# tyfeld/MMaDA-Parallel

Hardware: NVIDIA H100
Metric: denoised_tokens_per_sec (higher is better)
Workload: dtype bf16; 1 GPU; MMaDA-Parallel-A 8B, 1 prompt per GPU, 512x512 (1024 VQ tokens) + 256 text tokens, timesteps=64, text_steps=128, cfg_img=4.0, cfg_scale=0, temperature=1.0, text_temperature=0 (BASELINE configs[1]); seq_len=2414, parallelism=replicas x1 (independent prompts, no collective), weights=synthetic normal(0, 0.02) bf16, seeded, l2=16.2 GB of weights streamed per forward >> 50 MB L2 (no flush needed)

## Files before the change

mmada_parallel_b200/csrc/attention.cu:

```cuda
#include "mmdp_internal.h"
#include "ptx.cuh"

#include <stdlib.h>

#include <map>
#include <mutex>
#include <utility>

namespace mmdp {

static constexpr int kAttnThreads = 384;
static constexpr int kQBytes = 128 * 128 * 2;
template <int BKV> struct AttnCfg {
    static constexpr int kKBytes = BKV * 128 * 2;
    static constexpr int kVBytes = 128 * BKV * 2;
    static constexpr int kSmem = kQBytes + 2 * (kKBytes + kVBytes) + 1024  + 256 ;
};

__device__ __forceinline__ float ex2_approx(float x) {
    float y;
    asm("ex2.approx.ftz.f32 %0, %1;" : "=f"(y) : "f"(x));
    return y;
}

struct AttnSegs {
    int n;
    int start[kMaxSegs + 1];
    int tile0[kMaxSegs + 1];
};

struct AttnWin {
    AttnSegs segs;
    int q0[kMaxSegs], nq[kMaxSegs], out0[kMaxSegs];
};

template <int kBKV, bool kPacked, bool kGqa = false, bool kWin = false>
__device__ __forceinline__ void attention_body(const CUtensorMap& tmQ, const CUtensorMap& tmK, const CUtensorMap& tmVt,
                                               __nv_bfloat16* __restrict__ out, int H, int L, int d_model, float scale_log2,
                                               int n_full, int splits, float* __restrict__ part_ws, int Lq, const AttnSegs* segs,
                                               int kv_group = 1, const AttnWin* win = nullptr) {
    constexpr int kKBytes = AttnCfg<kBKV>::kKBytes, kVBytes = AttnCfg<kBKV>::kVBytes;
    extern __shared__ uint8_t smem_raw[];
    uint8_t* smem = reinterpret_cast<uint8_t*>((reinterpret_cast<uintptr_t>(smem_raw) + 1023) & ~uintptr_t(1023));
    uint8_t* sQ = smem;
    uint8_t* sK = sQ + kQBytes;
    uint8_t* sV = sK + 2 * kKBytes;
    uint64_t* bars = reinterpret_cast<uint64_t*>(sV + 2 * kVBytes);
    uint64_t* q_full = bars + 0;
    uint64_t* k_full = bars + 1;
    uint64_t* k_empty = bars + 3;
    uint64_t* v_full = bars + 5;
    uint64_t* v_empty = bars + 7;

    const int warp = threadIdx.x >> 5, lane = threadIdx.x & 31, wg = warp >> 2;
    int n_qt = (Lq + 127) / 128;
    int n_kv_all = (L + kBKV - 1) / kBKV;
    int tile = blockIdx.x, piece = -1;
    if ((int)blockIdx.x >= n_full) {
        const int t = (int)blockIdx.x - n_full;
        tile = n_full + t / splits;
        piece = t - (t / splits) * splits;
    }
    int seg = 0, seg0 = 0, tl = tile, q0 = 0, o0 = 0;
    if constexpr (kPacked) {
        for (int i = 1; i < segs->n; ++i)
            if (tile >= segs->tile0[i]) seg = i;
        seg0 = segs->start[seg];
        L = Lq = segs->start[seg + 1] - seg0;
        o0 = seg0;
        if constexpr (kWin) {
            q0 = win->q0[seg];
            Lq = win->nq[seg];
            o0 = win->out0[seg];
        }
        n_qt = (Lq + 127) / 128;
        n_kv_all = (L + kBKV - 1) / kBKV;
        tl = tile - segs->tile0[seg];
    }
    const int qt = tl % n_qt, h = (tl / n_qt) % H, b = kPacked ? seg : tile / (n_qt * H);
    const int hk = kGqa ? h / kv_group : h, Hk = kGqa ? H / kv_group : H;
    int jb = 0, je = n_kv_all;
    if (piece >= 0) {
        const int per = (n_kv_all + splits - 1) / splits;
        jb = piece * per;
        je = (jb + per < n_kv_all) ? jb + per : n_kv_all;
    }
    const int n_kv = je - jb;

    if (warp == 0 && lane == 0) {
        tma_prefetch_desc(&tmQ);
        tma_prefetch_desc(&tmK);
        tma_prefetch_desc(&tmVt);
        mbar_init(q_full, 1);
        for (int s = 0; s < 2; ++s) {
            mbar_init(&k_full[s], 1);
            mbar_init(&k_empty[s], 8);
            mbar_init(&v_full[s], 1);
            mbar_init(&v_empty[s], 8);
        }
        fence_barrier_init();
    }
    __syncthreads();
    pdl_launch_dependents();
    pdl_wait();

    if (wg == 0) {
        setmaxnreg_dec<40>();
        if (warp == 0 && elect_one_sync()) {
            const int qrow0 = (kPacked ? seg0 + q0 : b * Lq) + qt * 128;
            mbar_expect_tx(q_full, kQBytes);
            tma_load_2d(sQ, &tmQ, q_full, h * 128, qrow0);
            tma_load_2d(sQ + kQBytes / 2, &tmQ, q_full, h * 128 + 64, qrow0);
            for (int j = 0; j < n_kv; ++j) {
                const int st = j & 1;
                const uint32_t ph = (j >> 1) & 1;
                const int kv0 = (jb + j) * kBKV;
                mbar_wait(&k_empty[st], ph ^ 1);
                mbar_expect_tx(&k_full[st], kKBytes);
                tma_load_2d(sK + st * kKBytes, &tmK, &k_full[st], hk * 128, (kPacked ? seg0 : b * L) + kv0);
                tma_load_2d(sK + st * kKBytes + kKBytes / 2, &tmK, &k_full[st], hk * 128 + 64, (kPacked ? seg0 : b * L) + kv0);
                mbar_wait(&v_empty[st], ph ^ 1);
                mbar_expect_tx(&v_full[st], kVBytes);
                tma_load_2d(sV + st * kVBytes, &tmVt, &v_full[st], kv0, (b * Hk + hk) * 128);
                if (kBKV == 128) tma_load_2d(sV + st * kVBytes + kVBytes / 2, &tmVt, &v_full[st], kv0 + 64, (b * Hk + hk) * 128);
            }
        }
        __syncwarp();
        return;
    }

    setmaxnreg_inc<232>();
    const int half = wg - 1;
    const int r0 = half * 64 + (warp & 3) * 16 + (lane >> 2), c0 = 2 * (lane & 3);
    const uint32_t aQ = smem_u32(sQ) + half * (64 * 128);
    float o[64];
#pragma unroll
    for (int i = 0; i < 64; ++i) o[i] = 0.f;
    float m_run[2] = {-INFINITY, -INFINITY}, l_run[2] = {0.f, 0.f};
    mbar_wait(q_full, 0);
    for (int j = 0; j < n_kv; ++j) {
        const int st = j & 1;
        const uint32_t ph = (j >> 1) & 1;
        const int nvalid = L - (jb + j) * kBKV;
        float sacc[kBKV / 2];
        const uint32_t aK = smem_u32(sK + st * kKBytes);
        mbar_wait(&k_full[st], ph);
        wgmma_fence();
#pragma unroll
        for (int kk = 0; kk < 8; ++kk)
        {
            const uint64_t qd = smem_desc_kmajor_sw128(aQ + (kk >> 2) * (kQBytes / 2)) + (kk & 3) * 2;
            const uint64_t kd = smem_desc_kmajor_sw128(aK + (kk >> 2) * (kKBytes / 2)) + (kk & 3) * 2;
            if constexpr (kBKV == 128) wgmma_bf16_ss_n128(sacc, qd, kd, kk != 0);
            else wgmma_bf16_ss_n64(sacc, qd, kd, kk != 0);
        }
        wgmma_commit();
        wgmma_wait<0>();
        reg_fence(sacc);
        __syncwarp();
        if (lane == 0) mbar_arrive(&k_empty[st]);
        if (nvalid < kBKV) {
#pragma unroll
            for (int jj = 0; jj < kBKV / 8; ++jj)
#pragma unroll
                for (int e = 0; e < 2; ++e)
                    if (8 * jj + c0 + e >= nvalid) { sacc[4 * jj + e] = -INFINITY; sacc[4 * jj + 2 + e] = -INFINITY; }
        }
        float alpha[2], mneg[2];
#pragma unroll
        for (int hh = 0; hh < 2; ++hh) {
            float mx = sacc[2 * hh];
#pragma unroll
            for (int jj = 0; jj < kBKV / 8; ++jj) mx = fmaxf(mx, fmaxf(sacc[4 * jj + 2 * hh], sacc[4 * jj + 2 * hh + 1]));
            mx = fmaxf(mx, __shfl_xor_sync(0xffffffffu, mx, 1));
            mx = fmaxf(mx, __shfl_xor_sync(0xffffffffu, mx, 2));
            const float m_new = fmaxf(m_run[hh], mx);
            alpha[hh] = ex2_approx((m_run[hh] - m_new) * scale_log2);
            m_run[hh] = m_new;
            mneg[hh] = -m_new * scale_log2;
        }
        uint32_t pa[kBKV / 4];
        float rsum[2] = {0.f, 0.f};
#pragma unroll
        for (int jj = 0; jj < kBKV / 8; ++jj)
#pragma unroll
            for (int hh = 0; hh < 2; ++hh) {
                const float p0 = ex2_approx(fmaf(sacc[4 * jj + 2 * hh], scale_log2, mneg[hh]));
                const float p1 = ex2_approx(fmaf(sacc[4 * jj + 2 * hh + 1], scale_log2, mneg[hh]));
                rsum[hh] += p0 + p1;
                pa[2 * jj + hh] = pack_bf16x2(p0, p1);
            }
#pragma unroll
        for (int hh = 0; hh < 2; ++hh) l_run[hh] = fmaf(l_run[hh], alpha[hh], rsum[hh]);
#pragma unroll
        for (int jj = 0; jj < 16; ++jj) {
            o[4 * jj] *= alpha[0]; o[4 * jj + 1] *= alpha[0];
            o[4 * jj + 2] *= alpha[1]; o[4 * jj + 3] *= alpha[1];
        }
        const uint32_t aV = smem_u32(sV + st * kVBytes);
        mbar_wait(&v_full[st], ph);
        wgmma_fence();
#pragma unroll
        for (int kk = 0; kk < kBKV / 16; ++kk) {
            const uint32_t a[4] = {pa[4 * kk], pa[4 * kk + 1], pa[4 * kk + 2], pa[4 * kk + 3]};
            wgmma_bf16_rs_n128(o, a, smem_desc_kmajor_sw128(aV + (kk >> 2) * (kVBytes / 2)) + (kk & 3) * 2, 1);
        }
        wgmma_commit();
        wgmma_wait<0>();
        reg_fence(o);
        __syncwarp();
        if (lane == 0) mbar_arrive(&v_empty[st]);
    }
#pragma unroll
    for (int hh = 0; hh < 2; ++hh) {
        l_run[hh] += __shfl_xor_sync(0xffffffffu, l_run[hh], 1);
        l_run[hh] += __shfl_xor_sync(0xffffffffu, l_run[hh], 2);
    }
#pragma unroll
    for (int hh = 0; hh < 2; ++hh) {
        const int r = r0 + 8 * hh, qrow = qt * 128 + r;
        if (qrow >= Lq) continue;
        if (piece >= 0) {
            float* slot = part_ws + (size_t)((tile - n_full) * splits + piece) * (128 * 128 + 256);
            if ((lane & 3) == 0) {
                slot[128 * 128 + r] = m_run[hh];
                slot[128 * 128 + 128 + r] = l_run[hh];
            }
#pragma unroll
            for (int jj = 0; jj < 16; ++jj)
                *reinterpret_cast<float2*>(slot + (size_t)r * 128 + 8 * jj + c0) = make_float2(o[4 * jj + 2 * hh], o[4 * jj + 2 * hh + 1]);
        } else {
            const float inv_l = 1.0f / l_run[hh];
            __nv_bfloat16* orow = out + (size_t)((kPacked ? o0 : b * Lq) + qrow) * d_model + h * 128;
#pragma unroll
            for (int jj = 0; jj < 16; ++jj)
                *reinterpret_cast<uint32_t*>(orow + 8 * jj + c0) = pack_bf16x2(o[4 * jj + 2 * hh] * inv_l, o[4 * jj + 2 * hh + 1] * inv_l);
        }
    }
}

template <int kBKV>
__global__ void __launch_bounds__(kAttnThreads, 1)
attention_kernel(const __grid_constant__ CUtensorMap tmQ, const __grid_constant__ CUtensorMap tmK,
                 const __grid_constant__ CUtensorMap tmVt, __nv_bfloat16* __restrict__ out, int H, int L, int d_model,
                 float scale_log2, int n_full, int splits, float* __restrict__ part_ws, int Lq) {
    attention_body<kBKV, false>(tmQ, tmK, tmVt, out, H, L, d_model, scale_log2, n_full, splits, part_ws, Lq, nullptr);
}

template <int kBKV>
__global__ void __launch_bounds__(kAttnThreads, 1)
attention_packed_kernel(const __grid_constant__ CUtensorMap tmQ, const __grid_constant__ CUtensorMap tmK,
                        const __grid_constant__ CUtensorMap tmVt, __nv_bfloat16* __restrict__ out, int H, int d_model,
                        float scale_log2, int n_full, int splits, float* __restrict__ part_ws, const __grid_constant__ AttnSegs segs) {
    attention_body<kBKV, true>(tmQ, tmK, tmVt, out, H, 0, d_model, scale_log2, n_full, splits, part_ws, 0, &segs);
}

template <int kBKV>
__global__ void __launch_bounds__(kAttnThreads, 1)
attention_gqa_kernel(const __grid_constant__ CUtensorMap tmQ, const __grid_constant__ CUtensorMap tmK,
                     const __grid_constant__ CUtensorMap tmVt, __nv_bfloat16* __restrict__ out, int H, int L, int d_model,
                     float scale_log2, int n_full, int splits, float* __restrict__ part_ws, int Lq, int kv_group) {
    attention_body<kBKV, false, true>(tmQ, tmK, tmVt, out, H, L, d_model, scale_log2, n_full, splits, part_ws, Lq, nullptr, kv_group);
}

template <int kBKV>
__global__ void __launch_bounds__(kAttnThreads, 1)
attention_packed_gqa_kernel(const __grid_constant__ CUtensorMap tmQ, const __grid_constant__ CUtensorMap tmK,
                            const __grid_constant__ CUtensorMap tmVt, __nv_bfloat16* __restrict__ out, int H, int d_model,
                            float scale_log2, int n_full, int splits, float* __restrict__ part_ws, const __grid_constant__ AttnSegs segs,
                            int kv_group) {
    attention_body<kBKV, true, true>(tmQ, tmK, tmVt, out, H, 0, d_model, scale_log2, n_full, splits, part_ws, 0, &segs, kv_group);
}

template <int kBKV, bool kGqa>
__global__ void __launch_bounds__(kAttnThreads, 1)
attention_packed_window_kernel(const __grid_constant__ CUtensorMap tmQ, const __grid_constant__ CUtensorMap tmK,
                               const __grid_constant__ CUtensorMap tmVt, __nv_bfloat16* __restrict__ out, int H, int d_model,
                               float scale_log2, int n_full, int splits, float* __restrict__ part_ws, const __grid_constant__ AttnWin win,
                               int kv_group) {
    attention_body<kBKV, true, kGqa, true>(tmQ, tmK, tmVt, out, H, 0, d_model, scale_log2, n_full, splits, part_ws, 0, &win.segs,
                                           kv_group, &win);
}

template <bool kPacked, bool kWin = false>
__device__ __forceinline__ void attention_combine_body(const float* __restrict__ part_ws, __nv_bfloat16* __restrict__ out, int H,
                                                       int Lq, int d_model, float scale_log2, int n_full, int splits,
                                                       const AttnSegs* segs, const AttnWin* win = nullptr) {
    int n_qt = (Lq + 127) / 128;
    const int st = blockIdx.x, r = blockIdx.y, c = threadIdx.x;
    pdl_launch_dependents();
    pdl_wait();
    const int tile = n_full + st;
    int seg = 0, seg0 = 0, tl = tile;
    if constexpr (kPacked) {
        for (int i = 1; i < segs->n; ++i)
            if (tile >= segs->tile0[i]) seg = i;
        seg0 = segs->start[seg];
        Lq = segs->start[seg + 1] - seg0;
        if constexpr (kWin) {
            seg0 = win->out0[seg];
            Lq = win->nq[seg];
        }
        n_qt = (Lq + 127) / 128;
        tl = tile - segs->tile0[seg];
    }
    const int qt = tl % n_qt, h = (tl / n_qt) % H, b = kPacked ? seg : tile / (n_qt * H);
    const int qrow = qt * 128 + r;
    if (qrow >= Lq) return;
    const float* base = part_ws + (size_t)st * splits * (128 * 128 + 256);
    float m = -INFINITY;
    for (int i = 0; i < splits; ++i) m = fmaxf(m, base[(size_t)i * (128 * 128 + 256) + 128 * 128 + r]);
    float o = 0.f, l = 0.f;
    for (int i = 0; i < splits; ++i) {
        const float* slot = base + (size_t)i * (128 * 128 + 256);
        const float w = exp2f((slot[128 * 128 + r] - m) * scale_log2);
        o = fmaf(w, slot[(size_t)r * 128 + c], o);
        l = fmaf(w, slot[128 * 128 + 128 + r], l);
    }
    out[(size_t)((kPacked ? seg0 : b * Lq) + qrow) * d_model + h * 128 + c] = __float2bfloat16_rn(o / l);
}

__global__ void __launch_bounds__(128)
attention_combine_kernel(const float* __restrict__ part_ws, __nv_bfloat16* __restrict__ out, int H, int Lq, int d_model,
                         float scale_log2, int n_full, int splits) {
    attention_combine_body<false>(part_ws, out, H, Lq, d_model, scale_log2, n_full, splits, nullptr);
}

__global__ void __launch_bounds__(128)
attention_packed_combine_kernel(const float* __restrict__ part_ws, __nv_bfloat16* __restrict__ out, int H, int d_model,
                                float scale_log2, int n_full, int splits, const __grid_constant__ AttnSegs segs) {
    attention_combine_body<true>(part_ws, out, H, 0, d_model, scale_log2, n_full, splits, &segs);
}

__global__ void __launch_bounds__(128)
attention_packed_window_combine_kernel(const float* __restrict__ part_ws, __nv_bfloat16* __restrict__ out, int H, int d_model,
                                       float scale_log2, int n_full, int splits, const __grid_constant__ AttnWin win) {
    attention_combine_body<true, true>(part_ws, out, H, 0, d_model, scale_log2, n_full, splits, &win.segs, &win);
}

static std::map<std::pair<int, cudaStream_t>, std::pair<float*, size_t>> g_attn_ws;
static std::mutex g_attn_ws_mu;
static int attn_part_workspace(cudaStream_t stream, size_t need, float** out) {
    int dev = 0;
    MMDP_CUDA(cudaGetDevice(&dev));
    std::lock_guard<std::mutex> lk(g_attn_ws_mu);
    auto& e = g_attn_ws[std::make_pair(dev, stream)];
    if (need > e.second) {
        if (e.first) MMDP_CUDA(cudaFree(e.first));
        e.first = nullptr; e.second = 0;
        MMDP_CUDA(cudaMalloc(&e.first, need));
        e.second = need;
    }
    *out = e.first;
    return 0;
}

template <class KvbOf>
static void plan_split_tail(int tiles, KvbOf kvb_of, int& n_full, int& n_split, int& splits) {
    const int split_tail = opt(OPT_ATTN_SPLIT_TAIL), slots = num_sms();
    n_full = tiles; n_split = 0; splits = 1;
    auto fit_splits = [&](int want, int first) {
        int sp = want > 8 ? 8 : want;
        for (int t = first; t < tiles; ++t)
            if (sp > kvb_of(t) / 2) sp = kvb_of(t) / 2;
        auto empty_piece = [&](int s) {
            for (int t = first; t < tiles; ++t) {
                const int n_kvb = kvb_of(t);
                if ((s - 1) * ((n_kvb + s - 1) / s) >= n_kvb) return true;
            }
            return false;
        };
        while (sp >= 2 && empty_piece(sp)) --sp;
        return sp;
    };
    if (split_tail && tiles > slots && (tiles % slots) > 0 && (tiles % slots) * 4 <= slots) {
        n_split = tiles % slots;
        splits = fit_splits(slots / n_split, tiles - n_split);
        if (splits >= 2) n_full = tiles - n_split; else { n_split = 0; splits = 1; }
    } else if (split_tail && tiles * 2 <= slots) {
        splits = fit_splits(slots / tiles, 0);
        if (splits >= 2) { n_split = tiles; n_full = 0; } else splits = 1;
    }
}

template <class Kernel>
static int attn_smem_attr(Kernel kernel, int smem, unsigned long long& attr_set) {
    int dev = 0;
    MMDP_CUDA(cudaGetDevice(&dev));
    if (!(attr_set >> (dev & 63) & 1ull)) {
        MMDP_CUDA(cudaFuncSetAttribute(kernel, cudaFuncAttributeMaxDynamicSharedMemorySize, smem));
        attr_set |= 1ull << (dev & 63);
    }
    return 0;
}

template <int kBKV>
static int attention_launch(const __nv_bfloat16* q, const __nv_bfloat16* k, const __nv_bfloat16* vt, __nv_bfloat16* out, int B, int H,
                            int L, int Lpad, float scale, cudaStream_t stream, int Lq, int Hkv) {
    constexpr int kAttnSmem = AttnCfg<kBKV>::kSmem;
    if (B <= 0 || H <= 0 || L <= 0) return set_error("attention: empty problem");
    if (Lq <= 0) Lq = L;
    if (Hkv <= 0) Hkv = H;
    if (Hkv > H || H % Hkv) return set_error("attention: n_kv_heads=%d must divide n_heads=%d", Hkv, H);
    if (Lpad < L || (Lpad % 8)) return set_error("attention: Lpad must be >= L and a multiple of 8");
    const int d_model = H * 128, d_kv = Hkv * 128;
    CUtensorMap tmQ, tmK, tmVt;
    if (make_tmap_2d_bf16(&tmQ, q, (uint64_t)B * Lq, (uint64_t)d_model, (uint64_t)d_model, 128, 64)) return -1;
    if (make_tmap_2d_bf16(&tmK, k, (uint64_t)B * L, (uint64_t)d_kv, (uint64_t)d_kv, kBKV, 64)) return -1;
    if (make_tmap_2d_bf16(&tmVt, vt, (uint64_t)B * Hkv * 128, (uint64_t)Lpad, (uint64_t)Lpad, 128, 64)) return -1;
    const int n_qt = (Lq + 127) / 128, n_kvb = (L + kBKV - 1) / kBKV;
    const int tiles = n_qt * H * B;
    int n_full, n_split, splits;
    plan_split_tail(tiles, [&](int) { return n_kvb; }, n_full, n_split, splits);
    float* part_ws = nullptr;
    if (n_split > 0 && attn_part_workspace(stream, (size_t)n_split * splits * (128 * 128 + 256) * sizeof(float), &part_ws)) return -1;
    const int grid = n_full + n_split * splits;
    const float scale_log2 = scale * 1.4426950408889634f;
    const bool pdl = pdl_mode() != 0;
    LaunchScope ls(LK_ATTN, 4.0 * B * H * (double)Lq * L * 128, stream);
    if (Hkv != H) {
        static unsigned long long attr_set_gqa = 0;
        if (attn_smem_attr(attention_gqa_kernel<kBKV>, kAttnSmem, attr_set_gqa)) return -1;
        MMDP_CUDA(launch_ex(attention_gqa_kernel<kBKV>, dim3(grid), dim3(kAttnThreads), kAttnSmem, stream, pdl, false, tmQ, tmK, tmVt, out,
                            H, L, d_model, scale_log2, n_full, splits, part_ws, Lq, H / Hkv));
    } else {
        static unsigned long long attr_set = 0;
        if (attn_smem_attr(attention_kernel<kBKV>, kAttnSmem, attr_set)) return -1;
        MMDP_CUDA(launch_ex(attention_kernel<kBKV>, dim3(grid), dim3(kAttnThreads), kAttnSmem, stream, pdl, false, tmQ, tmK, tmVt, out, H, L,
                            d_model, scale_log2, n_full, splits, part_ws, Lq));
    }
    if (n_split > 0)
        MMDP_CUDA(launch_ex(attention_combine_kernel, dim3(n_split, 128), dim3(128), 0, stream, pdl, false, (const float*)part_ws, out, H, Lq,
                            d_model, scale_log2, n_full, splits));
    return 0;
}

template <int kBKV>
static int attention_packed_launch(const __nv_bfloat16* q, const __nv_bfloat16* k, const __nv_bfloat16* vt, __nv_bfloat16* out,
                                   const SegTable& segs, int H, int Lpad, float scale, cudaStream_t stream, int Hkv,
                                   const int* win_lo, const int* win_hi) {
    constexpr int kAttnSmem = AttnCfg<kBKV>::kSmem;
    if (segs.n <= 0 || segs.n > kMaxSegs || H <= 0) return set_error("attention_packed: %d sequences (1 to %d)", segs.n, kMaxSegs);
    if (Hkv <= 0) Hkv = H;
    if (Hkv > H || H % Hkv) return set_error("attention_packed: n_kv_heads=%d must divide n_heads=%d", Hkv, H);
    if (Lpad % 8) return set_error("attention_packed: Lpad must be a multiple of 8");
    if (!win_lo != !win_hi) return set_error("attention_packed: give both window bounds or neither");
    const bool windowed = win_lo != nullptr;
    AttnWin aw{};
    AttnSegs& as = aw.segs;
    as.n = segs.n;
    double work = 0;
    int Mq = 0;
    for (int s = 0; s <= segs.n; ++s) {
        as.start[s] = segs.start[s];
        if (s == segs.n) break;
        const int len = segs.start[s + 1] - segs.start[s];
        if (len <= 0 || len > Lpad) return set_error("attention_packed: sequence %d has length %d (Lpad %d)", s, len, Lpad);
        const int lo = windowed ? win_lo[s] : 0, hi = windowed ? win_hi[s] : len;
        if (lo < 0 || lo >= hi || hi > len)
            return set_error("attention_packed: sequence %d of length %d has the row window [%d, %d)", s, len, lo, hi);
        aw.q0[s] = lo;
        aw.nq[s] = hi - lo;
        aw.out0[s] = Mq;
        Mq += hi - lo;
        as.tile0[s + 1] = as.tile0[s] + (hi - lo + 127) / 128 * H;
        work += 4.0 * H * (double)(hi - lo) * len * 128;
    }
    const int M = segs.start[segs.n], tiles = as.tile0[segs.n], d_model = H * 128, d_kv = Hkv * 128;
    CUtensorMap tmQ, tmK, tmVt;
    if (make_tmap_2d_bf16(&tmQ, q, (uint64_t)M, (uint64_t)d_model, (uint64_t)d_model, 128, 64)) return -1;
    if (make_tmap_2d_bf16(&tmK, k, (uint64_t)M, (uint64_t)d_kv, (uint64_t)d_kv, kBKV, 64)) return -1;
    if (make_tmap_2d_bf16(&tmVt, vt, (uint64_t)segs.n * Hkv * 128, (uint64_t)Lpad, (uint64_t)Lpad, 128, 64)) return -1;
    auto kvb_of = [&](int t) {
        int s = 0;
        while (s + 1 < segs.n && t >= as.tile0[s + 1]) ++s;
        return (segs.start[s + 1] - segs.start[s] + kBKV - 1) / kBKV;
    };
    int n_full, n_split, splits;
    plan_split_tail(tiles, kvb_of, n_full, n_split, splits);
    float* part_ws = nullptr;
    if (n_split > 0 && attn_part_workspace(stream, (size_t)n_split * splits * (128 * 128 + 256) * sizeof(float), &part_ws)) return -1;
    const int grid = n_full + n_split * splits;
    const float scale_log2 = scale * 1.4426950408889634f;
    const bool pdl = pdl_mode() != 0;
    LaunchScope ls(LK_ATTN, work, stream);
    if (windowed) {
        auto kernel = Hkv != H ? attention_packed_window_kernel<kBKV, true> : attention_packed_window_kernel<kBKV, false>;
        static unsigned long long attr_set_win[2] = {0, 0};
        if (attn_smem_attr(kernel, kAttnSmem, attr_set_win[Hkv != H])) return -1;
        MMDP_CUDA(launch_ex(kernel, dim3(grid), dim3(kAttnThreads), kAttnSmem, stream, pdl, false, tmQ, tmK, tmVt, out, H, d_model,
                            scale_log2, n_full, splits, part_ws, aw, H / Hkv));
        if (n_split > 0)
            MMDP_CUDA(launch_ex(attention_packed_window_combine_kernel, dim3(n_split, 128), dim3(128), 0, stream, pdl, false,
                                (const float*)part_ws, out, H, d_model, scale_log2, n_full, splits, aw));
        return 0;
    }
    if (Hkv != H) {
        static unsigned long long attr_set_gqa = 0;
        if (attn_smem_attr(attention_packed_gqa_kernel<kBKV>, kAttnSmem, attr_set_gqa)) return -1;
        MMDP_CUDA(launch_ex(attention_packed_gqa_kernel<kBKV>, dim3(grid), dim3(kAttnThreads), kAttnSmem, stream, pdl, false, tmQ, tmK, tmVt,
                            out, H, d_model, scale_log2, n_full, splits, part_ws, as, H / Hkv));
    } else {
        static unsigned long long attr_set = 0;
        if (attn_smem_attr(attention_packed_kernel<kBKV>, kAttnSmem, attr_set)) return -1;
        MMDP_CUDA(launch_ex(attention_packed_kernel<kBKV>, dim3(grid), dim3(kAttnThreads), kAttnSmem, stream, pdl, false, tmQ, tmK, tmVt, out,
                            H, d_model, scale_log2, n_full, splits, part_ws, as));
    }
    if (n_split > 0)
        MMDP_CUDA(launch_ex(attention_packed_combine_kernel, dim3(n_split, 128), dim3(128), 0, stream, pdl, false, (const float*)part_ws,
                            out, H, d_model, scale_log2, n_full, splits, as));
    return 0;
}

int attention_fwd(const __nv_bfloat16* q, const __nv_bfloat16* k, const __nv_bfloat16* vt, __nv_bfloat16* out, int B, int H, int L,
                  int Lpad, float scale, cudaStream_t stream, int Lq, int Hkv) {
    const int version = opt(OPT_ATTN_VERSION);
    if (version == 7) return attention_launch<64>(q, k, vt, out, B, H, L, Lpad, scale, stream, Lq, Hkv);
    if (version != 6) return set_error("attention: unknown kernel generation %d (6 or 7)", version);
    return attention_launch<128>(q, k, vt, out, B, H, L, Lpad, scale, stream, Lq, Hkv);
}

int attention_packed_fwd(const __nv_bfloat16* q, const __nv_bfloat16* k, const __nv_bfloat16* vt, __nv_bfloat16* out,
                         const SegTable& segs, int H, int Lpad, float scale, cudaStream_t stream, int Hkv, const int* win_lo,
                         const int* win_hi) {
    const int version = opt(OPT_ATTN_VERSION);
    if (version == 7) return attention_packed_launch<64>(q, k, vt, out, segs, H, Lpad, scale, stream, Hkv, win_lo, win_hi);
    if (version != 6) return set_error("attention: unknown kernel generation %d (6 or 7)", version);
    return attention_packed_launch<128>(q, k, vt, out, segs, H, Lpad, scale, stream, Hkv, win_lo, win_hi);
}

}
```

mmada_parallel_b200/csrc/mmdp_internal.h:

```cpp
#pragma once
#include <cuda.h>
#include <cuda_bf16.h>
#include <cuda_runtime.h>
#include <stdint.h>
#include <stdio.h>

namespace mmdp {

enum Epilogue { EPI_PLAIN = 0, EPI_RESID = 1, EPI_QKVROPE = 2, EPI_SWIGLU = 3, EPI_F32 = 4, EPI_QKVROPE_PACKED = 5,
                EPI_QKVGQA = 6, EPI_QKVGQA_PACKED = 7 };
constexpr bool epi_is_gqa(int epi) { return epi == EPI_QKVGQA || epi == EPI_QKVGQA_PACKED; }
constexpr bool epi_is_qkv(int epi) { return epi == EPI_QKVROPE || epi == EPI_QKVROPE_PACKED || epi_is_gqa(epi); }
constexpr bool epi_is_packed(int epi) { return epi == EPI_QKVROPE_PACKED || epi == EPI_QKVGQA_PACKED; }

static constexpr int kMaxSegs = 64;
struct SegTable {
    int n;
    int start[kMaxSegs + 1];
};

int set_error(const char* fmt, ...);
const char* last_error();
int num_sms();

enum LaunchKind { LK_GEMM = 0, LK_ATTN = 1, LK_ROW = 2, LK_SAMPLE = 3, LK_COUNT = 4 };
struct LaunchScope {
    LaunchScope(int kind, double work, cudaStream_t s);
    ~LaunchScope();
    int idx;
    cudaStream_t stream;
};
void prof_enable(int on);
int prof_summary(double* ms, double* work, long long* launches);
long long launch_count(int reset);

int pdl_mode();
void set_pdl_mode(int on);
int env_int(const char* name, int dflt);
enum OptId { OPT_PDL = 0, OPT_GEMM_SPLITK, OPT_GEMM_L2PF, OPT_GEMM_L2PF_MOD, OPT_GEMM_GROUP_M, OPT_ATTN_SPLIT_TAIL,
             OPT_RMSNORM_WARP, OPT_ROW_WINDOW, OPT_ATTN_VERSION, OPT_GEMM_PAIR, OPT_COUNT };
int opt(int id);
int set_opt(const char* key, int value);

template <typename... KArgs, typename... Args>
inline cudaError_t launch_ex(void (*kernel)(KArgs...), dim3 grid, dim3 block, size_t smem, cudaStream_t stream, bool pdl,
                             bool coop, Args&&... args) {
    cudaLaunchConfig_t cfg{};
    cfg.gridDim = grid;
    cfg.blockDim = block;
    cfg.dynamicSmemBytes = smem;
    cfg.stream = stream;
    cudaLaunchAttribute at[2];
    unsigned n = 0;
    if (pdl) {
        at[n].id = cudaLaunchAttributeProgrammaticStreamSerialization;
        at[n].val.programmaticStreamSerializationAllowed = 1;
        ++n;
    }
    if (coop) {
        at[n].id = cudaLaunchAttributeCooperative;
        at[n].val.cooperative = 1;
        ++n;
    }
    cfg.attrs = at;
    cfg.numAttrs = n;
    return cudaLaunchKernelEx(&cfg, kernel, static_cast<KArgs>(args)...);
}

#define MMDP_CUDA(expr)                                                                              \
    do {                                                                                             \
        cudaError_t _e = (expr);                                                                     \
        if (_e != cudaSuccess)                                                                       \
            return ::mmdp::set_error("%s:%d: %s -> %s", __FILE__, __LINE__, #expr, cudaGetErrorString(_e)); \
    } while (0)

int make_tmap_2d_bf16(CUtensorMap* out, const void* base, uint64_t rows, uint64_t cols, uint64_t ld, uint32_t box_rows,
                      uint32_t box_cols);
int make_tmap_2d(CUtensorMap* out, const void* base, int elem_bytes, uint64_t rows, uint64_t cols, uint64_t ld,
                 uint32_t box_rows, uint32_t box_cols);

int conv_tf32(const float* A, int lda, long long a_rows, const float* W, int M, int N, int K, int T, const int* shifts,
              float* C, int ldc, const float* R, int ldr, const float* bias, int bias_along_m, float alpha, int pad_w,
              int pad_h, int scatter_w, int scatter_h, cudaStream_t stream);
int gn_swish(const float* x, float* y, int B, int C, int H, int W, double* stats_ws, const float* gamma, const float* beta,
             float eps, int swish, int compact, cudaStream_t stream);
int upsample2x(const float* x, float* y, int B, int C, int H, int W, cudaStream_t stream);
int softmax_rows_ld(float* s, int rows, int n, int ld, cudaStream_t stream);
int zero_border(float* y, int B, int C, int H, int W, cudaStream_t stream);
int lfq_to_padded(const int64_t* ids, float* z, int B, int H, int W, int bits, int Cpad, cudaStream_t stream);
int nchw_to_padded(const float* x, float* y, int B, int C, int Cpad, int H, int W, cudaStream_t stream);
int downsample_pick(const float* src, float* dst, int B, int C, int H, int W, cudaStream_t stream);
int lfq_indices(const float* z, int64_t* ids, int B, int h, int w, int bits, int ld, cudaStream_t stream);
int padded_to_nchw(const float* x, float* y, int B, int C, int ld, int H, int W, cudaStream_t stream);
int codebook_to_padded(const int64_t* ids, const float* cb, float* z, int B, int h, int w, int C, int Cpad, int64_t n_codes,
                       int* err, cudaStream_t stream);
int vq_nearest(const float* z, const float* cb, int B, int C, int h, int w, int n_codes, int64_t* ids, float* zq,
               cudaStream_t stream);

struct QkvRopeArgs {
    __nv_bfloat16* q;
    __nv_bfloat16* k;
    __nv_bfloat16* vt;
    const float* cos_tab;
    const float* sin_tab;
    int L, Lpad, d_model, n_heads;
    const int* pos_map = nullptr;
    int Tq = 0;
    int chunked = 0;
    int row0 = 0;
    const int2* seg_pos = nullptr;
    int n_kv_heads = 0;
    const __nv_bfloat16* bias = nullptr;
};

int packed_row_map(const SegTable& segs, int2* seg_pos, cudaStream_t stream);

struct GemmScatter {
    float* dst[8];
    int rows_per_rank, slot;
};

int gemm_bf16(int epi, const __nv_bfloat16* A, int lda, const __nv_bfloat16* W, int ldw, int M, int N, int K,
              __nv_bfloat16* C, int ldc, const __nv_bfloat16* resid, int ldr, const QkvRopeArgs* qa,
              cudaStream_t stream, const GemmScatter* sc = nullptr);

int gemm_group_m(int M);

int quantize_fp8(const __nv_bfloat16* x, int ldx, int rows, int K, int group, uint8_t* q, int ldq, float* scales,
                 cudaStream_t stream);
int gemm_fp8(int epi, const uint8_t* A, int lda, const float* sa, const uint8_t* W, int ldw, const float* sw, int M, int N,
             int K, __nv_bfloat16* C, int ldc, const __nv_bfloat16* resid, int ldr, const QkvRopeArgs* qa, cudaStream_t stream,
             const GemmScatter* scat = nullptr);

int gemm_pair_mode();
void set_gemm_pair_mode(int on);
int gemm_splitk_mode();
void set_gemm_splitk_mode(int mode);

int attention_fwd(const __nv_bfloat16* q, const __nv_bfloat16* k, const __nv_bfloat16* vt, __nv_bfloat16* out, int B,
                  int H, int L, int Lpad, float scale, cudaStream_t stream, int Lq = 0, int Hkv = 0);
int attention_packed_fwd(const __nv_bfloat16* q, const __nv_bfloat16* k, const __nv_bfloat16* vt, __nv_bfloat16* out,
                         const SegTable& segs, int H, int Lpad, float scale, cudaStream_t stream, int Hkv = 0,
                         const int* win_lo = nullptr, const int* win_hi = nullptr);

int embed_rows(const int64_t* ids, const __nv_bfloat16* wte, __nv_bfloat16* x, int M, int d, int64_t vocab,
               cudaStream_t stream, int* err = nullptr);
int rmsnorm(const __nv_bfloat16* x, int ldx, const __nv_bfloat16* w, __nv_bfloat16* y, int ldy, int M, int d, float eps,
            cudaStream_t stream);
int resid_add_f32(__nv_bfloat16* x, int ldx, const float* partial, int ldp, int M, int d, cudaStream_t stream);
int rmsnorm_rows(const __nv_bfloat16* x, int ldx, const int* rows, const __nv_bfloat16* w, __nv_bfloat16* y, int ldy,
                 int M, int d, float eps, cudaStream_t stream, int src_rows = 0x7fffffff, int* err = nullptr, int row_lo = 0, int row_hi = 0, int row_mod = 0);

int text_step(const __nv_bfloat16* cond, const __nv_bfloat16* uncond, int64_t ld, int R, int V, float text_cfg,
              const __nv_bfloat16* unoise, int64_t ld_noise, float temperature, int64_t* ids_text, int64_t mask_id,
              int k, int64_t* x0_ws, double* conf_ws, cudaStream_t stream, const double* unoise64 = nullptr);
int image_step(int variant, const __nv_bfloat16* cond, const __nv_bfloat16* unc_a, const __nv_bfloat16* unc_b, int64_t ld,
               int N, int C, float s_a, float s_b, const __nv_bfloat16* qnoise, const __nv_bfloat16* conf_noise,
               float temp, int sched_len, int64_t* ids, const int* pos, int64_t mask_id, int64_t vq_offset,
               int32_t* sampled_ws, float* selp_ws, uint8_t* unknown_ws, __nv_bfloat16* probs_out,
               int32_t* mask_len_out, uint8_t* masking_out, cudaStream_t stream);
int image_remask(int variant, int N, const int32_t* sampled, const float* selp, const uint8_t* unknown,
                 const __nv_bfloat16* conf_noise, float temp, int sched_len, int64_t* ids, const int* pos, int64_t mask_id,
                 int64_t vq_offset, int32_t* mask_len_out, uint8_t* masking_out, cudaStream_t stream, int k_direct = -1);
int image_step_t2i(const __nv_bfloat16* cond, const __nv_bfloat16* uncond, int64_t ld, int N, int C, float cfg,
                   const __nv_bfloat16* gumbel_u, float tau, const __nv_bfloat16* conf_u, float temperature, int keep_n,
                   int64_t* ids, const int* pos, int64_t mask_id, int64_t vq_offset, int32_t* sampled_ws, float* selp_ws,
                   uint8_t* unknown_ws, uint8_t* masking_out, cudaStream_t stream);
int lfq_decode(const int64_t* ids, float* zq, int B, int N, int bits, cudaStream_t stream);
int tp_reduce_norm(const float* recv_local, int rows_per_rank, int n_src, uint16_t* const* xn, uint32_t* const* flags, int n_ranks,
                   int my_rank, uint16_t* x_shard, const uint16_t* w, int row0, int nrows, int d, float eps, uint32_t epoch,
                   unsigned int* done_counter, cudaStream_t stream);
int tp_reduce_norm_fp8(const float* recv_local, int rows_per_rank, int n_src, uint8_t* const* xq, float* const* xs, int ld_s,
                       uint32_t* const* flags, int n_ranks, int my_rank, uint16_t* x_shard, const uint16_t* w, int row0, int nrows,
                       int d, float eps, uint32_t epoch, unsigned int* done_counter, cudaStream_t stream);

}
```

mmada_parallel_b200/csrc/runtime.cu:

```cuda
#include "mmdp_internal.h"

#include <stdarg.h>
#include <stdlib.h>
#include <string.h>

#include <mutex>
#include <unordered_map>
#include <vector>

namespace mmdp {

static thread_local char g_err[1024] = "";

int set_error(const char* fmt, ...) {
    va_list ap;
    va_start(ap, fmt);
    vsnprintf(g_err, sizeof(g_err), fmt, ap);
    va_end(ap);
    return -1;
}
const char* last_error() { return g_err; }

int num_sms() {
    static int n = 0;
    if (n == 0) {
        int dev = 0;
        cudaDeviceProp prop;
        if (cudaGetDevice(&dev) != cudaSuccess || cudaGetDeviceProperties(&prop, dev) != cudaSuccess) return 132;
        n = prop.multiProcessorCount;
    }
    return n;
}

int env_int(const char* name, int dflt) {
    const char* e = getenv(name);
    return (e && *e) ? atoi(e) : dflt;
}

struct Opt { const char* key; const char* env; int dflt; int val; bool init; };
static Opt g_opts[OPT_COUNT] = {
    {"pdl", "MMDP_PDL", 1, 0, false},
    {"gemm_splitk", "MMDP_GEMM_SPLITK", 2, 0, false},
    {"gemm_l2pf", "MMDP_GEMM_L2PF", 0, 0, false},
    {"gemm_l2pf_mod", "MMDP_GEMM_L2PF_MOD", 4, 0, false},
    {"gemm_group_m", "MMDP_GEMM_GROUP_M", -1, 0, false},
    {"attn_split_tail", "MMDP_ATTN_SPLIT_TAIL", 1, 0, false},
    {"rmsnorm_warp", "MMDP_RMSNORM_WARP", 1, 0, false},
    {"row_window", "MMDP_ROW_WINDOW", 1, 0, false},
    {"attn_version", "MMDP_ATTN_VERSION", 6, 0, false},
    {"gemm_pair", "MMDP_GEMM_PAIR", 0, 0, false},
};
int opt(int id) {
    Opt& o = g_opts[id];
    if (!o.init) { o.val = env_int(o.env, o.dflt); o.init = true; }
    return o.val;
}
int set_opt(const char* key, int value) {
    for (int i = 0; i < OPT_COUNT; ++i)
        if (!strcmp(g_opts[i].key, key)) { g_opts[i].val = value; g_opts[i].init = true; return 0; }
    return set_error("mmdp_set_option: unknown option '%s'", key);
}
int pdl_mode() { return opt(OPT_PDL) ? 1 : 0; }
void set_pdl_mode(int on) { set_opt("pdl", on ? 1 : 0); }

struct ProfRec { cudaEvent_t e0, e1; int kind; double work; };
static std::vector<ProfRec> g_prof;
static size_t g_prof_used = 0;
static bool g_prof_on = false;
static long long g_launches = 0;

LaunchScope::LaunchScope(int kind, double work, cudaStream_t s) : idx(-1), stream(s) {
    ++g_launches;
    if (!g_prof_on) return;
    if (g_prof_used == g_prof.size()) {
        ProfRec r{};
        if (cudaEventCreate(&r.e0) != cudaSuccess || cudaEventCreate(&r.e1) != cudaSuccess) return;
        g_prof.push_back(r);
    }
    idx = (int)g_prof_used++;
    g_prof[idx].kind = kind;
    g_prof[idx].work = work;
    cudaEventRecord(g_prof[idx].e0, s);
}
LaunchScope::~LaunchScope() {
    if (idx >= 0) cudaEventRecord(g_prof[idx].e1, stream);
}
void prof_enable(int on) {
    g_prof_on = on != 0;
    g_prof_used = 0;
}
int prof_summary(double* ms, double* work, long long* launches) {
    MMDP_CUDA(cudaDeviceSynchronize());
    for (int k = 0; k < LK_COUNT; ++k) { ms[k] = 0; work[k] = 0; launches[k] = 0; }
    for (size_t i = 0; i < g_prof_used; ++i) {
        float t = 0.f;
        MMDP_CUDA(cudaEventElapsedTime(&t, g_prof[i].e0, g_prof[i].e1));
        ms[g_prof[i].kind] += t;
        work[g_prof[i].kind] += g_prof[i].work;
        launches[g_prof[i].kind] += 1;
    }
    return 0;
}
long long launch_count(int reset) {
    long long v = g_launches;
    if (reset) g_launches = 0;
    return v;
}

typedef CUresult (*EncodeTiledFn)(CUtensorMap*, CUtensorMapDataType, cuuint32_t, void*, const cuuint64_t*,
                                  const cuuint64_t*, const cuuint32_t*, const cuuint32_t*, CUtensorMapInterleave,
                                  CUtensorMapSwizzle, CUtensorMapL2promotion, CUtensorMapFloatOOBfill);

static EncodeTiledFn encode_fn() {
    static EncodeTiledFn fn = nullptr;
    if (!fn) {
        void* p = nullptr;
        cudaDriverEntryPointQueryResult qres;
        if (cudaGetDriverEntryPoint("cuTensorMapEncodeTiled", &p, cudaEnableDefault, &qres) != cudaSuccess ||
            qres != cudaDriverEntryPointSuccess)
            return nullptr;
        fn = reinterpret_cast<EncodeTiledFn>(p);
    }
    return fn;
}

int make_tmap_2d_bf16(CUtensorMap* out, const void* base, uint64_t rows, uint64_t cols, uint64_t ld, uint32_t box_rows,
                      uint32_t box_cols) {
    return make_tmap_2d(out, base, 2, rows, cols, ld, box_rows, box_cols);
}

struct TmapKey {
    const void* base;
    uint64_t rows, cols, ld;
    uint32_t box_rows, box_cols;
    int elem_bytes;
    bool operator==(const TmapKey& o) const {
        return base == o.base && rows == o.rows && cols == o.cols && ld == o.ld && box_rows == o.box_rows &&
               box_cols == o.box_cols && elem_bytes == o.elem_bytes;
    }
};
struct TmapKeyHash {
    size_t operator()(const TmapKey& k) const {
        uint64_t h = reinterpret_cast<uint64_t>(k.base) * 0x9E3779B97F4A7C15ull;
        h ^= (k.rows + 0x9E3779B97F4A7C15ull + (h << 6) + (h >> 2));
        h ^= (k.cols * 0xC2B2AE3D27D4EB4Full + (h << 6) + (h >> 2));
        h ^= (k.ld + ((uint64_t)k.box_rows << 32) + ((uint64_t)k.box_cols << 8) + (uint64_t)k.elem_bytes + (h << 6) + (h >> 2));
        return (size_t)h;
    }
};
static std::unordered_map<TmapKey, CUtensorMap, TmapKeyHash> g_tmaps;
static std::mutex g_tmap_mu;

int make_tmap_2d(CUtensorMap* out, const void* base, int elem_bytes, uint64_t rows, uint64_t cols, uint64_t ld,
                 uint32_t box_rows, uint32_t box_cols) {
    EncodeTiledFn fn = encode_fn();
    if (!fn) return set_error("cuTensorMapEncodeTiled not available (no CUDA driver / no GPU)");
    if (elem_bytes != 1 && elem_bytes != 2 && elem_bytes != 4) return set_error("tmap: element size must be 1 (e4m3), 2 (bf16) or 4 (fp32)");
    if (box_cols * (uint32_t)elem_bytes != 128) return set_error("tmap: box must be exactly one 128-byte swizzle atom wide");
    if (box_rows == 0 || box_rows > 256) return set_error("tmap: box_rows out of range");
    const TmapKey key{base, rows, cols, ld, box_rows, box_cols, elem_bytes};
    {
        std::lock_guard<std::mutex> lk(g_tmap_mu);
        auto it = g_tmaps.find(key);
        if (it != g_tmaps.end()) {
            *out = it->second;
            return 0;
        }
    }
    cuuint64_t gdim[2] = {cols, rows};
    cuuint64_t gstride[1] = {ld * (uint64_t)elem_bytes};
    cuuint32_t box[2] = {box_cols, box_rows};
    cuuint32_t estr[2] = {1, 1};
    const CUtensorMapDataType dt = elem_bytes == 1 ? CU_TENSOR_MAP_DATA_TYPE_UINT8
                                   : (elem_bytes == 2 ? CU_TENSOR_MAP_DATA_TYPE_BFLOAT16 : CU_TENSOR_MAP_DATA_TYPE_FLOAT32);
    CUresult r = fn(out, dt, 2, const_cast<void*>(base), gdim, gstride, box, estr,
                    CU_TENSOR_MAP_INTERLEAVE_NONE, CU_TENSOR_MAP_SWIZZLE_128B, CU_TENSOR_MAP_L2_PROMOTION_L2_256B,
                    CU_TENSOR_MAP_FLOAT_OOB_FILL_NONE);
    if (r != CUDA_SUCCESS)
        return set_error("cuTensorMapEncodeTiled failed (%d) base=%p rows=%llu cols=%llu ld=%llu box=[%u,%u]", (int)r,
                         base, (unsigned long long)rows, (unsigned long long)cols, (unsigned long long)ld, box_rows,
                         box_cols);
    {
        std::lock_guard<std::mutex> lk(g_tmap_mu);
        if (g_tmaps.size() >= 8192) g_tmaps.clear();
        g_tmaps.emplace(key, *out);
    }
    return 0;
}

}
```

Baseline: 106.4 tokens/s.

## Overlap QK^T of next KV tile with PV of current tile in attention

Adds a software-pipelined attention consumer path that issues the next tile's S=QK^T wgmma while the current PV wgmma runs, then does softmax between the waits. This hides softmax and wgmma latency behind tensor core work. Register split is shifted toward consumers (24/240) to hold the extra S and P arrays. A spin-limited barrier wait traps on hang. The path is enabled by default through a new option, and attention is only part of a forward pass that is dominated by streaming weights.

New measurement: 107.4 tokens/s (median of 6 runs). About the same (+0.9%).

```diff
diff --git a/mmada_parallel_b200/csrc/attention.cu b/mmada_parallel_b200/csrc/attention.cu
--- a/mmada_parallel_b200/csrc/attention.cu
+++ b/mmada_parallel_b200/csrc/attention.cu
@@ -34,7 +34,79 @@
     int q0[kMaxSegs], nq[kMaxSegs], out0[kMaxSegs];
 };
 
-template <int kBKV, bool kPacked, bool kGqa = false, bool kWin = false>
+__device__ __forceinline__ void mbar_wait_flag(uint64_t* bar, uint32_t parity, bool& hung) {
+    uint32_t spins = 0;
+    while (!mbar_try_wait(bar, parity))
+        if (++spins > MMDP_WAIT_SPIN_LIMIT) { hung = true; break; }
+}
+
+template <int kBKV>
+__device__ __forceinline__ void attn_issue_s(float (&sacc)[kBKV / 2], uint32_t aQ, uint32_t aK) {
+#pragma unroll
+    for (int kk = 0; kk < 8; ++kk) {
+        const uint64_t qd = smem_desc_kmajor_sw128(aQ + (kk >> 2) * (kQBytes / 2)) + (kk & 3) * 2;
+        const uint64_t kd = smem_desc_kmajor_sw128(aK + (kk >> 2) * (AttnCfg<kBKV>::kKBytes / 2)) + (kk & 3) * 2;
+        if constexpr (kBKV == 128) wgmma_bf16_ss_n128(sacc, qd, kd, kk != 0);
+        else wgmma_bf16_ss_n64(sacc, qd, kd, kk != 0);
+    }
+}
+
+template <int kBKV>
+__device__ __forceinline__ void attn_issue_pv(float (&o)[64], const uint32_t (&pa)[kBKV / 4], uint32_t aV) {
+#pragma unroll
+    for (int kk = 0; kk < kBKV / 16; ++kk) {
+        const uint32_t a[4] = {pa[4 * kk], pa[4 * kk + 1], pa[4 * kk + 2], pa[4 * kk + 3]};
+        wgmma_bf16_rs_n128(o, a, smem_desc_kmajor_sw128(aV + (kk >> 2) * (AttnCfg<kBKV>::kVBytes / 2)) + (kk & 3) * 2, 1);
+    }
+}
+
+template <int kBKV>
+__device__ __forceinline__ void attn_softmax(float (&sacc)[kBKV / 2], int nvalid, int c0, float scale_log2, float (&m_run)[2],
+                                             float (&l_run)[2], float (&alpha)[2]) {
+    if (nvalid < kBKV) {
+#pragma unroll
+        for (int jj = 0; jj < kBKV / 8; ++jj)
+#pragma unroll
+            for (int e = 0; e < 2; ++e)
+                if (8 * jj + c0 + e >= nvalid) { sacc[4 * jj + e] = -INFINITY; sacc[4 * jj + 2 + e] = -INFINITY; }
+    }
+    float mneg[2];
+#pragma unroll
+    for (int hh = 0; hh < 2; ++hh) {
+        float mx = sacc[2 * hh];
+#pragma unroll
+        for (int jj = 0; jj < kBKV / 8; ++jj) mx = fmaxf(mx, fmaxf(sacc[4 * jj + 2 * hh], sacc[4 * jj + 2 * hh + 1]));
+        mx = fmaxf(mx, __shfl_xor_sync(0xffffffffu, mx, 1));
+        mx = fmaxf(mx, __shfl_xor_sync(0xffffffffu, mx, 2));
+        const float m_new = fmaxf(m_run[hh], mx);
+        alpha[hh] = ex2_approx((m_run[hh] - m_new) * scale_log2);
+        m_run[hh] = m_new;
+        mneg[hh] = -m_new * scale_log2;
+    }
+    float rsum[2] = {0.f, 0.f};
+#pragma unroll
+    for (int jj = 0; jj < kBKV / 8; ++jj)
+#pragma unroll
+        for (int hh = 0; hh < 2; ++hh) {
+            const float p0 = ex2_approx(fmaf(sacc[4 * jj + 2 * hh], scale_log2, mneg[hh]));
+            const float p1 = ex2_approx(fmaf(sacc[4 * jj + 2 * hh + 1], scale_log2, mneg[hh]));
+            rsum[hh] += p0 + p1;
+            sacc[4 * jj + 2 * hh] = p0;
+            sacc[4 * jj + 2 * hh + 1] = p1;
+        }
+#pragma unroll
+    for (int hh = 0; hh < 2; ++hh) l_run[hh] = fmaf(l_run[hh], alpha[hh], rsum[hh]);
+}
+
+template <int kBKV>
+__device__ __forceinline__ void attn_pack_p(uint32_t (&pa)[kBKV / 4], const float (&sacc)[kBKV / 2]) {
+#pragma unroll
+    for (int jj = 0; jj < kBKV / 8; ++jj)
+#pragma unroll
+        for (int hh = 0; hh < 2; ++hh) pa[2 * jj + hh] = pack_bf16x2(sacc[4 * jj + 2 * hh], sacc[4 * jj + 2 * hh + 1]);
+}
+
+template <int kBKV, bool kPacked, bool kGqa = false, bool kWin = false, bool kPipe = false>
 __device__ __forceinline__ void attention_body(const CUtensorMap& tmQ, const CUtensorMap& tmK, const CUtensorMap& tmVt,
                                                __nv_bfloat16* __restrict__ out, int H, int L, int d_model, float scale_log2,
                                                int n_full, int splits, float* __restrict__ part_ws, int Lq, const AttnSegs* segs,
@@ -105,7 +177,8 @@
     pdl_wait();
 
     if (wg == 0) {
-        setmaxnreg_dec<40>();
+        if constexpr (kPipe) setmaxnreg_dec<24>();
+        else setmaxnreg_dec<40>();
         if (warp == 0 && elect_one_sync()) {
             const int qrow0 = (kPacked ? seg0 + q0 : b * Lq) + qt * 128;
             mbar_expect_tx(q_full, kQBytes);
@@ -129,7 +202,8 @@
         return;
     }
 
-    setmaxnreg_inc<232>();
+    if constexpr (kPipe) setmaxnreg_inc<240>();
+    else setmaxnreg_inc<232>();
     const int half = wg - 1;
     const int r0 = half * 64 + (warp & 3) * 16 + (lane >> 2), c0 = 2 * (lane & 3);
     const uint32_t aQ = smem_u32(sQ) + half * (64 * 128);
@@ -137,6 +211,68 @@
 #pragma unroll
     for (int i = 0; i < 64; ++i) o[i] = 0.f;
     float m_run[2] = {-INFINITY, -INFINITY}, l_run[2] = {0.f, 0.f};
+    if constexpr (kPipe) {
+        float sacc[kBKV / 2];
+        uint32_t pa[kBKV / 4];
+        float alpha[2];
+        bool hung = false;
+        mbar_wait_flag(q_full, 0, hung);
+        mbar_wait_flag(&k_full[0], 0, hung);
+        wgmma_fence();
+        attn_issue_s<kBKV>(sacc, aQ, smem_u32(sK));
+        wgmma_commit();
+        wgmma_wait<0>();
+        reg_fence(sacc);
+        __syncwarp();
+        if (lane == 0) mbar_arrive(&k_empty[0]);
+        attn_softmax<kBKV>(sacc, L - jb * kBKV, c0, scale_log2, m_run, l_run, alpha);
+        attn_pack_p<kBKV>(pa, sacc);
+        for (int j = 0; j + 1 < n_kv; ++j) {
+            const int st = j & 1, sn = st ^ 1;
+            const uint32_t ph = (j >> 1) & 1, phn = ((j + 1) >> 1) & 1;
+#pragma unroll
+            for (int jj = 0; jj < 16; ++jj) {
+                o[4 * jj] *= alpha[0]; o[4 * jj + 1] *= alpha[0];
+                o[4 * jj + 2] *= alpha[1]; o[4 * jj + 3] *= alpha[1];
+            }
+            mbar_wait_flag(&k_full[sn], phn, hung);
+            wgmma_fence();
+            attn_issue_s<kBKV>(sacc, aQ, smem_u32(sK + sn * kKBytes));
+            wgmma_commit();
+            mbar_wait_flag(&v_full[st], ph, hung);
+            wgmma_fence();
+            attn_issue_pv<kBKV>(o, pa, smem_u32(sV + st * kVBytes));
+            wgmma_commit();
+            wgmma_wait<1>();
+            reg_fence(sacc);
+            __syncwarp();
+            if (lane == 0) mbar_arrive(&k_empty[sn]);
+            attn_softmax<kBKV>(sacc, L - (jb + j + 1) * kBKV, c0, scale_log2, m_run, l_run, alpha);
+            wgmma_wait<0>();
+            reg_fence(o);
+            __syncwarp();
+            if (lane == 0) mbar_arrive(&v_empty[st]);
+            attn_pack_p<kBKV>(pa, sacc);
+        }
+        {
+            const int j = n_kv - 1, st = j & 1;
+            const uint32_t ph = (j >> 1) & 1;
+#pragma unroll
+            for (int jj = 0; jj < 16; ++jj) {
+                o[4 * jj] *= alpha[0]; o[4 * jj + 1] *= alpha[0];
+                o[4 * jj + 2] *= alpha[1]; o[4 * jj + 3] *= alpha[1];
+            }
+            mbar_wait_flag(&v_full[st], ph, hung);
+            wgmma_fence();
+            attn_issue_pv<kBKV>(o, pa, smem_u32(sV + st * kVBytes));
+            wgmma_commit();
+            wgmma_wait<0>();
+            reg_fence(o);
+            __syncwarp();
+            if (lane == 0) mbar_arrive(&v_empty[st]);
+        }
+        if (hung) __trap();
+    } else {
     mbar_wait(q_full, 0);
     for (int j = 0; j < n_kv; ++j) {
         const int st = j & 1;
@@ -211,6 +347,7 @@
         __syncwarp();
         if (lane == 0) mbar_arrive(&v_empty[st]);
     }
+    }
 #pragma unroll
     for (int hh = 0; hh < 2; ++hh) {
         l_run[hh] += __shfl_xor_sync(0xffffffffu, l_run[hh], 1);
@@ -239,46 +376,46 @@
     }
 }
 
-template <int kBKV>
+template <int kBKV, bool kPipe>
 __global__ void __launch_bounds__(kAttnThreads, 1)
 attention_kernel(const __grid_constant__ CUtensorMap tmQ, const __grid_constant__ CUtensorMap tmK,
                  const __grid_constant__ CUtensorMap tmVt, __nv_bfloat16* __restrict__ out, int H, int L, int d_model,
                  float scale_log2, int n_full, int splits, float* __restrict__ part_ws, int Lq) {
-    attention_body<kBKV, false>(tmQ, tmK, tmVt, out, H, L, d_model, scale_log2, n_full, splits, part_ws, Lq, nullptr);
-}
-
-template <int kBKV>
+    attention_body<kBKV, false, false, false, kPipe>(tmQ, tmK, tmVt, out, H, L, d_model, scale_log2, n_full, splits, part_ws, Lq, nullptr);
+}
+
+template <int kBKV, bool kPipe>
 __global__ void __launch_bounds__(kAttnThreads, 1)
 attention_packed_kernel(const __grid_constant__ CUtensorMap tmQ, const __grid_constant__ CUtensorMap tmK,
                         const __grid_constant__ CUtensorMap tmVt, __nv_bfloat16* __restrict__ out, int H, int d_model,
                         float scale_log2, int n_full, int splits, float* __restrict__ part_ws, const __grid_constant__ AttnSegs segs) {
-    attention_body<kBKV, true>(tmQ, tmK, tmVt, out, H, 0, d_model, scale_log2, n_full, splits, part_ws, 0, &segs);
-}
-
-template <int kBKV>
+    attention_body<kBKV, true, false, false, kPipe>(tmQ, tmK, tmVt, out, H, 0, d_model, scale_log2, n_full, splits, part_ws, 0, &segs);
+}
+
+template <int kBKV, bool kPipe>
 __global__ void __launch_bounds__(kAttnThreads, 1)
 attention_gqa_kernel(const __grid_constant__ CUtensorMap tmQ, const __grid_constant__ CUtensorMap tmK,
                      const __grid_constant__ CUtensorMap tmVt, __nv_bfloat16* __restrict__ out, int H, int L, int d_model,
                      float scale_log2, int n_full, int splits, float* __restrict__ part_ws, int Lq, int kv_group) {
-    attention_body<kBKV, false, true>(tmQ, tmK, tmVt, out, H, L, d_model, scale_log2, n_full, splits, part_ws, Lq, nullptr, kv_group);
-}
-
-template <int kBKV>
+    attention_body<kBKV, false, true, false, kPipe>(tmQ, tmK, tmVt, out, H, L, d_model, scale_log2, n_full, splits, part_ws, Lq, nullptr, kv_group);
+}
+
+template <int kBKV, bool kPipe>
 __global__ void __launch_bounds__(kAttnThreads, 1)
 attention_packed_gqa_kernel(const __grid_constant__ CUtensorMap tmQ, const __grid_constant__ CUtensorMap tmK,
                             const __grid_constant__ CUtensorMap tmVt, __nv_bfloat16* __restrict__ out, int H, int d_model,
                             float scale_log2, int n_full, int splits, float* __restrict__ part_ws, const __grid_constant__ AttnSegs segs,
                             int kv_group) {
-    attention_body<kBKV, true, true>(tmQ, tmK, tmVt, out, H, 0, d_model, scale_log2, n_full, splits, part_ws, 0, &segs, kv_group);
-}
-
-template <int kBKV, bool kGqa>
+    attention_body<kBKV, true, true, false, kPipe>(tmQ, tmK, tmVt, out, H, 0, d_model, scale_log2, n_full, splits, part_ws, 0, &segs, kv_group);
+}
+
+template <int kBKV, bool kGqa, bool kPipe>
 __global__ void __launch_bounds__(kAttnThreads, 1)
 attention_packed_window_kernel(const __grid_constant__ CUtensorMap tmQ, const __grid_constant__ CUtensorMap tmK,
                                const __grid_constant__ CUtensorMap tmVt, __nv_bfloat16* __restrict__ out, int H, int d_model,
                                float scale_log2, int n_full, int splits, float* __restrict__ part_ws, const __grid_constant__ AttnWin win,
                                int kv_group) {
-    attention_body<kBKV, true, kGqa, true>(tmQ, tmK, tmVt, out, H, 0, d_model, scale_log2, n_full, splits, part_ws, 0, &win.segs,
+    attention_body<kBKV, true, kGqa, true, kPipe>(tmQ, tmK, tmVt, out, H, 0, d_model, scale_log2, n_full, splits, part_ws, 0, &win.segs,
                                            kv_group, &win);
 }
 
@@ -417,16 +554,19 @@
     const int grid = n_full + n_split * splits;
     const float scale_log2 = scale * 1.4426950408889634f;
     const bool pdl = pdl_mode() != 0;
+    const int pipe = opt(OPT_ATTN_PIPELINE) != 0;
     LaunchScope ls(LK_ATTN, 4.0 * B * H * (double)Lq * L * 128, stream);
     if (Hkv != H) {
-        static unsigned long long attr_set_gqa = 0;
-        if (attn_smem_attr(attention_gqa_kernel<kBKV>, kAttnSmem, attr_set_gqa)) return -1;
-        MMDP_CUDA(launch_ex(attention_gqa_kernel<kBKV>, dim3(grid), dim3(kAttnThreads), kAttnSmem, stream, pdl, false, tmQ, tmK, tmVt, out,
+        auto kernel = pipe ? attention_gqa_kernel<kBKV, true> : attention_gqa_kernel<kBKV, false>;
+        static unsigned long long attr_set_gqa[2] = {0, 0};
+        if (attn_smem_attr(kernel, kAttnSmem, attr_set_gqa[pipe])) return -1;
+        MMDP_CUDA(launch_ex(kernel, dim3(grid), dim3(kAttnThreads), kAttnSmem, stream, pdl, false, tmQ, tmK, tmVt, out,
                             H, L, d_model, scale_log2, n_full, splits, part_ws, Lq, H / Hkv));
     } else {
-        static unsigned long long attr_set = 0;
-        if (attn_smem_attr(attention_kernel<kBKV>, kAttnSmem, attr_set)) return -1;
-        MMDP_CUDA(launch_ex(attention_kernel<kBKV>, dim3(grid), dim3(kAttnThreads), kAttnSmem, stream, pdl, false, tmQ, tmK, tmVt, out, H, L,
+        auto kernel = pipe ? attention_kernel<kBKV, true> : attention_kernel<kBKV, false>;
+        static unsigned long long attr_set[2] = {0, 0};
+        if (attn_smem_attr(kernel, kAttnSmem, attr_set[pipe])) return -1;
+        MMDP_CUDA(launch_ex(kernel, dim3(grid), dim3(kAttnThreads), kAttnSmem, stream, pdl, false, tmQ, tmK, tmVt, out, H, L,
                             d_model, scale_log2, n_full, splits, part_ws, Lq));
     }
     if (n_split > 0)
@@ -483,11 +623,13 @@
     const int grid = n_full + n_split * splits;
     const float scale_log2 = scale * 1.4426950408889634f;
     const bool pdl = pdl_mode() != 0;
+    const int pipe = opt(OPT_ATTN_PIPELINE) != 0;
     LaunchScope ls(LK_ATTN, work, stream);
     if (windowed) {
-        auto kernel = Hkv != H ? attention_packed_window_kernel<kBKV, true> : attention_packed_window_kernel<kBKV, false>;
-        static unsigned long long attr_set_win[2] = {0, 0};
-        if (attn_smem_attr(kernel, kAttnSmem, attr_set_win[Hkv != H])) return -1;
+        auto kernel = Hkv != H ? (pipe ? attention_packed_window_kernel<kBKV, true, true> : attention_packed_window_kernel<kBKV, true, false>)
+                               : (pipe ? attention_packed_window_kernel<kBKV, false, true> : attention_packed_window_kernel<kBKV, false, false>);
+        static unsigned long long attr_set_win[2][2] = {{0, 0}, {0, 0}};
+        if (attn_smem_attr(kernel, kAttnSmem, attr_set_win[pipe][Hkv != H])) return -1;
         MMDP_CUDA(launch_ex(kernel, dim3(grid), dim3(kAttnThreads), kAttnSmem, stream, pdl, false, tmQ, tmK, tmVt, out, H, d_model,
                             scale_log2, n_full, splits, part_ws, aw, H / Hkv));
         if (n_split > 0)
@@ -496,14 +638,16 @@
         return 0;
     }
     if (Hkv != H) {
-        static unsigned long long attr_set_gqa = 0;
-        if (attn_smem_attr(attention_packed_gqa_kernel<kBKV>, kAttnSmem, attr_set_gqa)) return -1;
-        MMDP_CUDA(launch_ex(attention_packed_gqa_kernel<kBKV>, dim3(grid), dim3(kAttnThreads), kAttnSmem, stream, pdl, false, tmQ, tmK, tmVt,
+        auto kernel = pipe ? attention_packed_gqa_kernel<kBKV, true> : attention_packed_gqa_kernel<kBKV, false>;
+        static unsigned long long attr_set_gqa[2] = {0, 0};
+        if (attn_smem_attr(kernel, kAttnSmem, attr_set_gqa[pipe])) return -1;
+        MMDP_CUDA(launch_ex(kernel, dim3(grid), dim3(kAttnThreads), kAttnSmem, stream, pdl, false, tmQ, tmK, tmVt,
                             out, H, d_model, scale_log2, n_full, splits, part_ws, as, H / Hkv));
     } else {
-        static unsigned long long attr_set = 0;
-        if (attn_smem_attr(attention_packed_kernel<kBKV>, kAttnSmem, attr_set)) return -1;
-        MMDP_CUDA(launch_ex(attention_packed_kernel<kBKV>, dim3(grid), dim3(kAttnThreads), kAttnSmem, stream, pdl, false, tmQ, tmK, tmVt, out,
+        auto kernel = pipe ? attention_packed_kernel<kBKV, true> : attention_packed_kernel<kBKV, false>;
+        static unsigned long long attr_set[2] = {0, 0};
+        if (attn_smem_attr(kernel, kAttnSmem, attr_set[pipe])) return -1;
+        MMDP_CUDA(launch_ex(kernel, dim3(grid), dim3(kAttnThreads), kAttnSmem, stream, pdl, false, tmQ, tmK, tmVt, out,
                             H, d_model, scale_log2, n_full, splits, part_ws, as));
     }
     if (n_split > 0)
diff --git a/mmada_parallel_b200/csrc/mmdp_internal.h b/mmada_parallel_b200/csrc/mmdp_internal.h
--- a/mmada_parallel_b200/csrc/mmdp_internal.h
+++ b/mmada_parallel_b200/csrc/mmdp_internal.h
@@ -38,7 +38,7 @@
 void set_pdl_mode(int on);
 int env_int(const char* name, int dflt);
 enum OptId { OPT_PDL = 0, OPT_GEMM_SPLITK, OPT_GEMM_L2PF, OPT_GEMM_L2PF_MOD, OPT_GEMM_GROUP_M, OPT_ATTN_SPLIT_TAIL,
-             OPT_RMSNORM_WARP, OPT_ROW_WINDOW, OPT_ATTN_VERSION, OPT_GEMM_PAIR, OPT_COUNT };
+             OPT_RMSNORM_WARP, OPT_ROW_WINDOW, OPT_ATTN_VERSION, OPT_ATTN_PIPELINE, OPT_GEMM_PAIR, OPT_COUNT };
 int opt(int id);
 int set_opt(const char* key, int value);
 
diff --git a/mmada_parallel_b200/csrc/runtime.cu b/mmada_parallel_b200/csrc/runtime.cu
--- a/mmada_parallel_b200/csrc/runtime.cu
+++ b/mmada_parallel_b200/csrc/runtime.cu
@@ -48,6 +48,7 @@
     {"rmsnorm_warp", "MMDP_RMSNORM_WARP", 1, 0, false},
     {"row_window", "MMDP_ROW_WINDOW", 1, 0, false},
     {"attn_version", "MMDP_ATTN_VERSION", 6, 0, false},
+    {"attn_pipeline", "MMDP_ATTN_PIPELINE", 1, 0, false},
     {"gemm_pair", "MMDP_GEMM_PAIR", 0, 0, false},
 };
 int opt(int id) {
```
